# quantscious/finmlkit

Hardware: AMD Instinct MI355X
Metric: ticks/sec aggregated to bars (higher is better)
Workload: dtype f64

## Files before the change

finmlkit_amd/csrc/fmk_median.h:

```cpp
#pragma once
#include <math.h>

#include "fmk_common.h"
#include "fmk_dpp.h"

template <bool AF64> struct MedKey;
template <> struct MedKey<false> {
    typedef uint32_t K;
    static constexpr int BITS = 32;
    static constexpr K MAXK = 0xFFFFFFFFu;
    static constexpr K KEY_NEG_INF = 0x007FFFFFu;
    static constexpr K KEY_POS_INF = 0xFF800000u;
    __device__ static __forceinline__ K tokey(K u) { return (u & 0x80000000u) ? ~u : (u | 0x80000000u); }
    __device__ static __forceinline__ K load(const void *p, int64_t j) { return tokey(((const uint32_t *)p)[j]); }
    __device__ static __forceinline__ double value(K k)
    {
        uint32_t u = (k & 0x80000000u) ? (k & 0x7FFFFFFFu) : ~k;
        return (double)__uint_as_float(u);
    }
};
template <> struct MedKey<true> {
    typedef uint64_t K;
    static constexpr int BITS = 64;
    static constexpr K MAXK = 0xFFFFFFFFFFFFFFFFull;
    static constexpr K KEY_NEG_INF = 0x000FFFFFFFFFFFFFull;
    static constexpr K KEY_POS_INF = 0xFFF0000000000000ull;
    __device__ static __forceinline__ K tokey(K u) { return (u >> 63) ? ~u : (u | 0x8000000000000000ull); }
    __device__ static __forceinline__ K load(const void *p, int64_t j) { return tokey(((const uint64_t *)p)[j]); }
    __device__ static __forceinline__ double value(K k)
    {
        uint64_t u = (k >> 63) ? (k & 0x7FFFFFFFFFFFFFFFull) : ~k;
        return __longlong_as_double((long long)u);
    }
};

__device__ __forceinline__ int med_popc(bool p) { return __popcll(__ballot(p)); }

template <typename K>
__device__ __forceinline__ K med_wave_umin(K v)
{
#pragma unroll
    for (int o = 32; o > 0; o >>= 1) { K w = __shfl_xor(v, o, 64); v = w < v ? w : v; }
    return v;
}
template <typename K>
__device__ __forceinline__ K med_wave_umax(K v)
{
#pragma unroll
    for (int o = 32; o > 0; o >>= 1) { K w = __shfl_xor(v, o, 64); v = w > v ? w : v; }
    return v;
}

template <typename K>
__device__ __forceinline__ K med_bitonic64(K v, int lane)
{
#pragma unroll
    for (int k = 2; k <= 64; k <<= 1) {
#pragma unroll
        for (int j = k >> 1; j > 0; j >>= 1) {
            K w = __shfl_xor(v, j, 64);
            bool up = (lane & k) == 0;
            bool lower = (lane & j) == 0;
            K mn = w < v ? w : v, mx = w < v ? v : w;
            v = (lower == up) ? mn : mx;
        }
    }
    return v;
}

template <bool AF64, int NREG, bool EXACT = false>
struct MedBar {
    typedef MedKey<AF64> MK;
    typedef typename MK::K K;
    K key[NREG > 0 ? NREG : 1];
    const void *amount;
    int64_t start, cnt;
    int lane;

    __device__ __forceinline__ void load_all()
    {
        if constexpr (NREG > 0) {
            K raw[NREG];
#pragma unroll
            for (int r = 0; r < NREG; ++r) {
                const int64_t j = (int64_t)r * 64 + lane;
                raw[r] = 0;
                if (j < cnt) raw[r] = ((const K *)amount)[start + j];
            }
#pragma unroll
            for (int r = 0; r < NREG; ++r) asm volatile("" : "+v"(raw[r]));
#pragma unroll
            for (int r = 0; r < NREG; ++r) {
                const int64_t j = (int64_t)r * 64 + lane;
                key[r] = j < cnt ? MK::tokey(raw[r]) : MK::MAXK;
            }
        }
    }
    __device__ __forceinline__ bool maybe_invalid(int r) const { return !EXACT || r == NREG - 1; }
    __device__ __forceinline__ void minmax(K &mn, K &mx)
    {
        K a = MK::MAXK, b = 0;
        if constexpr (NREG > 0) {
#pragma unroll
            for (int r = 0; r < NREG; ++r) {
                const K k = key[r];
                a = k < a ? k : a;
                if (maybe_invalid(r)) b = (k != MK::MAXK && k > b) ? k : b;
                else b = k > b ? k : b;
            }
        } else {
            for (int64_t j = lane; j < cnt; j += 64) {
                K k = MK::load(amount, start + j);
                a = k < a ? k : a;
                b = k > b ? k : b;
            }
        }
        mn = med_wave_umin<K>(a);
        mx = med_wave_umax<K>(b);
    }
    __device__ __forceinline__ int64_t count_le(K pivot)
    {
        if constexpr (NREG > 0) {
            int c = 0;
#pragma unroll
            for (int r = 0; r < NREG; ++r) c += med_popc(key[r] <= pivot);
            return c;
        } else {
            int64_t c = 0;
            for (int64_t j = lane; j < cnt; j += 64) c += MK::load(amount, start + j) <= pivot;
            return fmk_wave_sum(c);
        }
    }
    __device__ __forceinline__ void split(K pivot, K &below, K &above)
    {
        K a = 0, b = MK::MAXK;
        if constexpr (NREG > 0) {
#pragma unroll
            for (int r = 0; r < NREG; ++r) {
                const K k = key[r];
                a = (k <= pivot && k > a) ? k : a;
                b = (k > pivot && k < b) ? k : b;
            }
        } else {
            for (int64_t j = lane; j < cnt; j += 64) {
                K k = MK::load(amount, start + j);
                a = (k <= pivot && k > a) ? k : a;
                b = (k > pivot && k < b) ? k : b;
            }
        }
        below = med_wave_umax<K>(a);
        above = med_wave_umin<K>(b);
    }
    __device__ __forceinline__ void inside_minmax(K lo, K hi, K &mn, K &mx)
    {
        K a = MK::MAXK, b = 0;
#pragma unroll
        for (int r = 0; r < (NREG > 0 ? NREG : 1); ++r) {
            const K k = key[r];
            const bool in = k > lo && k <= hi;
            a = (in && k < a) ? k : a;
            b = (in && k > b) ? k : b;
        }
        mn = med_wave_umin<K>(a);
        mx = med_wave_umax<K>(b);
    }
    __device__ __forceinline__ void compact(K lo, K hi, K *buf)
    {
        int base = 0;
        if constexpr (NREG > 0) {
#pragma unroll
            for (int r = 0; r < NREG; ++r) {
                K k = key[r];
                bool in = k > lo && k <= hi;
                uint64_t m = __ballot(in);
                int pos = base + __builtin_amdgcn_mbcnt_hi((uint32_t)(m >> 32), __builtin_amdgcn_mbcnt_lo((uint32_t)m, 0));
                if (in) buf[pos] = k;
                base += __popcll(m);
            }
        } else {
            for (int64_t j0 = 0; j0 < cnt; j0 += 64) {
                int64_t j = j0 + lane;
                K k = j < cnt ? MK::load(amount, start + j) : MK::MAXK;
                bool in = j < cnt && k > lo && k <= hi;
                uint64_t m = __ballot(in);
                int pos = base + __builtin_amdgcn_mbcnt_hi((uint32_t)(m >> 32), __builtin_amdgcn_mbcnt_lo((uint32_t)m, 0));
                if (in) buf[pos] = k;
                base += __popcll(m);
            }
        }
    }
};

template <bool AF64, int NREG, bool EXACT, bool SNAP = false>
__device__ __forceinline__ bool med_rank_pair(MedBar<AF64, NREG, EXACT> &bar, typename MedKey<AF64>::K *buf,
                                              int64_t k1, int64_t k2, typename MedKey<AF64>::K &v1,
                                              typename MedKey<AF64>::K &v2)
{
    typedef MedKey<AF64> MK;
    typedef typename MK::K K;
    const int lane = bar.lane;
    const int64_t cnt = bar.cnt;
    K mn, mx;
    bar.minmax(mn, mx);
    if (mn < MK::KEY_NEG_INF || mx > MK::KEY_POS_INF) return false;
    K lo = mn - 1, hi = mx;
    int64_t clo = 0, chi = cnt;
    for (int nstep = 0;; ++nstep) {
        if constexpr (SNAP && NREG > 0) {
            if (chi - clo > 64 && hi - lo > 1 && (nstep == 10 || nstep == 16 || nstep == 22)) {
                K mn_in, mx_in;
                bar.inside_minmax(lo, hi, mn_in, mx_in);
                hi = mx_in;
                lo = (mn_in == mx_in ? mx_in : mn_in) - 1;
                continue;
            }
        }
        if (chi - clo <= 64) {
            buf[lane] = MK::MAXK;
            __builtin_amdgcn_wave_barrier();
            bar.compact(lo, hi, buf);
            __builtin_amdgcn_wave_barrier();
            K v = med_bitonic64<K>(buf[lane], lane);
            __builtin_amdgcn_wave_barrier();
            v1 = __shfl(v, (int)(k1 - clo), 64);
            v2 = __shfl(v, (int)(k2 - clo), 64);
            break;
        }
        if (hi - lo == 1) { v1 = v2 = hi; break; }
        K pivot = lo + ((hi - lo) >> 1);
        int64_t c = bar.count_le(pivot);
        if (c > k2) { hi = pivot; chi = c; }
        else if (c <= k1) { lo = pivot; clo = c; }
        else {
            bar.split(pivot, v1, v2);
            break;
        }
    }
    return true;
}

template <bool AF64, int NREG, bool EXACT, bool SNAP = false>
__device__ __forceinline__ double med_search(MedBar<AF64, NREG, EXACT> &bar, typename MedKey<AF64>::K *buf)
{
    typedef MedKey<AF64> MK;
    typename MK::K v1, v2;
    const int64_t cnt = bar.cnt;
    if (!med_rank_pair<AF64, NREG, EXACT, SNAP>(bar, buf, (cnt - 1) >> 1, cnt >> 1, v1, v2)) return NAN;
    return (cnt & 1) ? MK::value(v1) : (MK::value(v1) + MK::value(v2)) / 2.0;
}

template <bool AF64, int NREG>
__device__ __forceinline__ double med_select(const void *amount, int64_t start, int64_t cnt, int lane,
                                             typename MedKey<AF64>::K *buf)
{
    MedBar<AF64, NREG, false> bar;
    bar.amount = amount; bar.start = start; bar.cnt = cnt; bar.lane = lane;
    bar.load_all();
    return med_search<AF64, NREG, false>(bar, buf);
}

#define MED_SEL_BITS 11
#define MED_SEL_BINS (1 << MED_SEL_BITS)
template <bool AF64, int THREADS>
__device__ __forceinline__ void med_block_select(const void *__restrict__ amount, int64_t start, int64_t cnt, int64_t rank0,
                                                 int64_t rank1, typename MedKey<AF64>::K &k1, typename MedKey<AF64>::K &k2,
                                                 bool &any_nan)
{
    typedef MedKey<AF64> MK;
    typedef typename MK::K K;
    constexpr int D = (MK::BITS + MED_SEL_BITS - 1) / MED_SEL_BITS;
    constexpr int PER = MED_SEL_BINS / THREADS;
    constexpr int NW = THREADS / 64;
    __shared__ unsigned hist[2][MED_SEL_BINS];
    __shared__ K s_prefix[2];
    __shared__ int64_t s_rank[2];
    __shared__ unsigned s_wsum[2][NW];
    __shared__ int s_nan;
    const int tid = threadIdx.x, lane = fmk_lane(), w = tid >> 6;
    __syncthreads();
    if (tid == 0) { s_prefix[0] = 0; s_prefix[1] = 0; s_rank[0] = rank0; s_rank[1] = rank1; s_nan = 0; }
    bool nan = false;
#pragma unroll 1
    for (int p = 0; p < D; ++p) {
#pragma unroll
        for (int q = 0; q < PER; ++q) { hist[0][tid + q * THREADS] = 0; hist[1][tid + q * THREADS] = 0; }
        __syncthreads();
        const K pre0 = s_prefix[0], pre1 = s_prefix[1];
        const int64_t rk0 = s_rank[0], rk1 = s_rank[1];
        const bool same = pre0 == pre1;
        const int rest = MK::BITS - MED_SEL_BITS * (p + 1);
        const int shift = rest > 0 ? rest : 0;
        const int width = rest >= 0 ? MED_SEL_BITS : MED_SEL_BITS + rest;
        const unsigned mask = (1u << width) - 1u;
        for (int64_t j = tid; j < cnt; j += THREADS) {
            const K k = MK::load(amount, start + j);
            if (p == 0) nan |= k < MK::KEY_NEG_INF || k > MK::KEY_POS_INF;
            const K hi = p == 0 ? (K)0 : (K)(k >> (shift + width));
            const unsigned d = (unsigned)(k >> shift) & mask;
            if (hi == pre0) atomicAdd(&hist[0][d], 1u);
            if (!same && hi == pre1) atomicAdd(&hist[1][d], 1u);
        }
        __syncthreads();
#pragma unroll
        for (int t = 0; t < 2; ++t) {
            const unsigned *hh = hist[same ? 0 : t];
            unsigned h[PER], tot = 0;
#pragma unroll
            for (int q = 0; q < PER; ++q) { h[q] = hh[tid * PER + q]; tot += h[q]; }
            unsigned inc = tot;
#pragma unroll
            for (int o = 1; o < 64; o <<= 1) { const unsigned v = __shfl_up(inc, o, 64); if (lane >= o) inc += v; }
            if (lane == 63) s_wsum[t][w] = inc;
            __syncthreads();
            unsigned base = 0;
            for (int k = 0; k < w; ++k) base += s_wsum[t][k];
            int64_t cum = (int64_t)base + inc - tot;
            const int64_t rk = t == 0 ? rk0 : rk1;
#pragma unroll
            for (int q = 0; q < PER; ++q) {
                if (cum <= rk && rk < cum + h[q]) {
                    s_prefix[t] = (K)(((t == 0 ? pre0 : pre1) << width) | (K)(tid * PER + q));
                    s_rank[t] = rk - cum;
                }
                cum += h[q];
            }
        }
        __syncthreads();
    }
    if (nan) s_nan = 1;
    __syncthreads();
    k1 = s_prefix[0]; k2 = s_prefix[1]; any_nan = s_nan != 0;
}

struct FuMed {
    uint32_t lo, hi;
    uint32_t width;
    int have;
};

__device__ __forceinline__ uint32_t fu_wave_umin(uint32_t v)
{
    return (uint32_t)fmk_dpp_reduce((int)(v ^ 0x80000000u), (int)0x7FFFFFFF, FmkOpMin()) ^ 0x80000000u;
}
__device__ __forceinline__ uint32_t fu_wave_umax(uint32_t v)
{
    return (uint32_t)fmk_dpp_reduce((int)(v ^ 0x80000000u), (int)0x80000000, FmkOpMax()) ^ 0x80000000u;
}

template <int R>
__device__ __forceinline__ double fu_median(const uint32_t (&key)[R], int cnt, int lane, bool maybe_nan, FuMed &med, uint32_t *buf)
{
    typedef MedKey<false> MK;
    const int k1 = (cnt - 1) >> 1, k2 = cnt >> 1;
    uint32_t lo = 0, hi = 0;
    int clo = 0, chi = cnt;
    bool inside = false;
    if (med.have && !maybe_nan) {
        int c1 = 0, c2 = 0;
#pragma unroll
        for (int i = 0; i < R; ++i) {
            c1 += med_popc(key[i] <= med.lo);
            c2 += med_popc(key[i] <= med.hi);
        }
        if (c1 <= k1 && k2 < c2) {
            inside = true; lo = med.lo; hi = med.hi; clo = c1; chi = c2;
            const int nc = c2 - c1;
            if (nc > 144) med.width -= med.width >> 2;
            else if (nc < 80) med.width += (med.width >> 2) + 1;
        }
    }
    if (!inside) {
        uint32_t a = MK::MAXK, bmax = 0;
#pragma unroll
        for (int i = 0; i < R; ++i) {
            const uint32_t k = key[i];
            a = k < a ? k : a;
            bmax = (k != MK::MAXK && k > bmax) ? k : bmax;
        }
        const uint32_t mn = fu_wave_umin(a), mx = fu_wave_umax(bmax);
        if (mn < MK::KEY_NEG_INF || mx > MK::KEY_POS_INF) { med.have = 0; return NAN; }
        lo = mn - 1; hi = mx; clo = 0; chi = cnt;
    }
    uint32_t v1 = 0, v2 = 0;
    bool found = false;
    while (chi - clo > 64) {
        if (hi - lo == 1) { v1 = v2 = hi; found = true; break; }
        const uint32_t pivot = lo + ((hi - lo) >> 1);
        int c = 0;
#pragma unroll
        for (int i = 0; i < R; ++i) c += med_popc(key[i] <= pivot);
        if (c > k2) { hi = pivot; chi = c; }
        else if (c <= k1) { lo = pivot; clo = c; }
        else {
            uint32_t a = 0, bb = MK::MAXK;
#pragma unroll
            for (int i = 0; i < R; ++i) {
                const uint32_t k = key[i];
                a = (k <= pivot && k > a) ? k : a;
                bb = (k > pivot && k < bb) ? k : bb;
            }
            v1 = fu_wave_umax(a); v2 = fu_wave_umin(bb);
            found = true;
            break;
        }
    }
    uint32_t cmin = 0, cmax = 0;
    if (!found) {
        buf[lane] = MK::MAXK;
        __builtin_amdgcn_wave_barrier();
        int base = 0;
#pragma unroll
        for (int i = 0; i < R; ++i) {
            const uint32_t k = key[i];
            const bool in = k > lo && k <= hi;
            const uint64_t m = __ballot(in);
            const int pos = base + (int)__builtin_amdgcn_mbcnt_hi((uint32_t)(m >> 32), __builtin_amdgcn_mbcnt_lo((uint32_t)m, 0));
            if (in) buf[pos] = k;
            base += __popcll(m);
        }
        __builtin_amdgcn_wave_barrier();
        const uint32_t c0 = buf[lane];
        __builtin_amdgcn_wave_barrier();
        if (!inside) {
            cmin = fu_wave_umin(c0);
            cmax = fu_wave_umax(lane < chi - clo ? c0 : 0u);
        }
        for (;;) {
            if (hi - lo == 1) { v1 = v2 = hi; break; }
            const uint32_t pivot = lo + ((hi - lo) >> 1);
            const int c = clo + med_popc(c0 <= pivot);
            if (c > k2) hi = pivot;
            else if (c <= k1) lo = pivot;
            else {
                v1 = fu_wave_umax(c0 <= pivot ? c0 : 0u);
                v2 = fu_wave_umin(c0 > pivot ? c0 : MK::MAXK);
                break;
            }
        }
    }
    if (!inside) {
        if (found) med.width = 64;
        else {
            const uint32_t wl = v1 - cmin, wh = cmax - v2;
            med.width = wl > wh ? wl : wh;
        }
        med.have = 1;
    }
    med.lo = v1 > med.width + 1 ? v1 - med.width - 1 : 0;
    med.hi = v2 < 0xFFFFFFFEu - med.width ? v2 + med.width : 0xFFFFFFFEu;
    return (cnt & 1) ? MK::value(v1) : (MK::value(v1) + MK::value(v2)) / 2.0;
}
```

finmlkit_amd/csrc/fmk_ohlcv.hip:

```cpp
#include <math.h>
#include <stdlib.h>

#include <utility>

#include "fmk_common.h"
#include "fmk_dpp.h"
#include "fmk_f32tie.h"
#include "fmk_median.h"

#define FMK_SMALL_NCH 21
#define FMK_PACKED_MAX_MEAN 64

struct OhlcvOut {
    double *open, *high, *low, *close;
    float *vol;
    double *vwap;
    int64_t *trades;
    double *median;
    unsigned long long *vol_redo;
};

__device__ __forceinline__ void ohlcv_empty(const OhlcvOut &o, int64_t b, const double *price, int64_t e, int64_t n)
{
    double p = price[fmk_wrap(e, n)];
// ... 89 lines not shown
        if constexpr (MED) {
            blo = brk[4 * q]; bhi = brk[4 * q + 1];
            mycand = cand + ((start - base) >> 2);
            cap = (int)((e - s) >> 2);
            if (tid == 0) { s_ncand = 0; s_nan = 0; }
            __syncthreads();
        }
        auto med_tick = [&](int64_t jj, bool in_bar) {
            if constexpr (MED) {
                const uint32_t raw = in_bar ? ((const uint32_t *)amount)[jj] : 0u;
                const uint32_t k = MedKey<false>::tokey(raw);
                nan |= in_bar && (k < MedKey<false>::KEY_NEG_INF || k > MedKey<false>::KEY_POS_INF);
                below += (in_bar && k < blo) ? 1 : 0;
                const bool inb = in_bar && k >= blo && k <= bhi;
                const uint64_t m = __ballot(inb);
                if (m) {
                    int base = 0;
                    if (lane == (int)__builtin_ctzll(m)) base = atomicAdd(&s_ncand, (int)__popcll(m));
                    base = __builtin_amdgcn_readlane(base, (int)__builtin_ctzll(m));
                    const int pos = base + (int)__builtin_amdgcn_mbcnt_hi((uint32_t)(m >> 32), __builtin_amdgcn_mbcnt_lo((uint32_t)m, 0));
                    if (inb && pos < cap) mycand[pos] = raw;
                }
            }
        };
        int64_t j = start + tid;
        for (; j + 3 * OH_WIDE_THREADS <= e; j += 4 * OH_WIDE_THREADS) {
            const double p0 = price[j], p1 = price[j + OH_WIDE_THREADS], p2 = price[j + 2 * OH_WIDE_THREADS],
                         p3 = price[j + 3 * OH_WIDE_THREADS];
            const double a0 = fmk_amt<AF64>(amount, j), a1 = fmk_amt<AF64>(amount, j + OH_WIDE_THREADS),
                         a2 = fmk_amt<AF64>(amount, j + 2 * OH_WIDE_THREADS), a3 = fmk_amt<AF64>(amount, j + 3 * OH_WIDE_THREADS);
            hi = fmax(fmax(hi, p0), fmax(p1, fmax(p2, p3)));
            lo = fmin(fmin(lo, p0), fmin(p1, fmin(p2, p3)));
            tv += a0; td += p0 * a0;
            tv += a1; td += p1 * a1;
            tv += a2; td += p2 * a2;
            tv += a3; td += p3 * a3;
            med_tick(j, true); med_tick(j + OH_WIDE_THREADS, true); med_tick(j + 2 * OH_WIDE_THREADS, true);
            med_tick(j + 3 * OH_WIDE_THREADS, true);
        }
        for (; j - tid <= e; j += OH_WIDE_THREADS) {
            const bool in_bar = j <= e;
            const int64_t jc = in_bar ? j : e;
            const double p0 = price[jc], a0 = in_bar ? fmk_amt<AF64>(amount, jc) : 0.0;
            hi = fmax(hi, p0);
            lo = fmin(lo, p0);
            tv += a0; td += in_bar ? p0 * a0 : 0.0;
            med_tick(jc, in_bar);
        }
        hi = fmk_dpp_reduce(hi, (double)-INFINITY, FmkOpMax());
        lo = fmk_dpp_reduce(lo, (double)INFINITY, FmkOpMin());
        tv = fmk_dpp_reduce(tv, 0.0, FmkOpAdd());
        td = fmk_dpp_reduce(td, 0.0, FmkOpAdd());
        if constexpr (MED) {
            below = fmk_dpp_reduce(below, (int64_t)0, FmkOpAdd());
            if (lane == 0) s_below[w] = below;
            if (__ballot(nan) != 0 && lane == 0) s_nan = 1;
        }
        if (lane == 0) { s_red[0][w] = hi; s_red[1][w] = lo; s_red[2][w] = tv; s_red[3][w] = td; }
        __syncthreads();
        if constexpr (MED) {
            if (tid == 0) {
                int64_t bl = 0;
                for (int k = 0; k < OH_WIDE_THREADS / 64; ++k) bl += s_below[k];
                res[3 * q] = bl; res[3 * q + 1] = s_ncand; res[3 * q + 2] = s_nan;
            }
        }
        if (w == 0) {
            hi = s_red[0][0]; lo = s_red[1][0]; tv = s_red[2][0]; td = s_red[3][0];
            for (int k = 1; k < OH_WIDE_THREADS / 64; ++k) {
                hi = fmax(hi, s_red[0][k]); lo = fmin(lo, s_red[1][k]); tv += s_red[2][k]; td += s_red[3][k];
            }
            ohlcv_finish<AF64>(o, b, price, start, e, hi, lo, tv, td, lane, true);
        }
        __syncthreads();
    }
}


struct OhlBracket { uint32_t blo, bhi; int ok; int pad; };
struct OhlCount { int64_t below; int64_t ncand; int64_t nan; };

__device__ __forceinline__ int ohl_stride(int64_t cnt) { return cnt <= 65536 ? 16 : (cnt <= ((int64_t)1 << 21) ? 64 : 256); }

__global__ __launch_bounds__(256) void k_bar_med_sample(const float *__restrict__ amount, const int64_t *__restrict__ ci,
                                                        const int64_t *__restrict__ list, const int *__restrict__ go,
                                                        float *__restrict__ samp, OhlBracket *__restrict__ brk, float g_scale,
                                                        int64_t base)
{
    if (go && *go == 0) return;
    const int64_t n_list = list[0];
    for (int64_t q = blockIdx.x; q < n_list; q += gridDim.x) {
        const int64_t b = list[1 + q], s0 = ci[b], e = ci[b + 1], start = s0 + 1, cnt = e - s0;
        const int stride = ohl_stride(cnt);
        const int64_t ns = cnt / stride;
        float *mine = samp + ((start - base) >> 4);
        for (int64_t j = threadIdx.x; j < ns; j += 256) mine[j] = amount[start + j * stride];
        __syncthreads();
        const int g = (int)(1.9f * g_scale * sqrtf((float)ns)) + 4;
        const int64_t r_lo = ns / 2 - g > 0 ? ns / 2 - g : 0, r_hi = ns / 2 + g < ns - 1 ? ns / 2 + g : ns - 1;
        uint32_t klo, khi;
        bool any_nan;
        med_block_select<false, 256>(mine, 0, ns, r_lo, r_hi, klo, khi, any_nan);
        if (threadIdx.x == 0) brk[q] = OhlBracket{klo, khi, any_nan ? 0 : 1, 0};
        __syncthreads();
    }
}

__global__ __launch_bounds__(256) void k_bar_med_finish(const int64_t *__restrict__ ci, const int64_t *__restrict__ list,
                                                        const int *__restrict__ go, const uint32_t *__restrict__ cand,
                                                        const OhlCount *__restrict__ res, int64_t *__restrict__ fallback,
                                                        double *__restrict__ o_median, int64_t base)
{
    if (go && *go == 0) return;
    typedef MedKey<false> MK;
    const int64_t n_list = list[0];
    for (int64_t q = blockIdx.x; q < n_list; q += gridDim.x) {
        const int64_t b = list[1 + q], s0 = ci[b], e = ci[b + 1], start = s0 + 1, cnt = e - s0;
        const OhlCount r = res[q];
        const int64_t k1 = (cnt - 1) >> 1, k2 = cnt >> 1, cap = cnt >> 2;
        if (r.nan) { if (threadIdx.x == 0) o_median[b] = NAN; continue; }
        if (!(r.below <= k1 && k2 < r.below + r.ncand && r.ncand <= cap)) {
            if (threadIdx.x == 0) fallback[1 + atomicAdd((unsigned long long *)fallback, 1ULL)] = b;
            continue;
        }
        uint32_t v1, v2;
        bool any_nan;
        med_block_select<false, 256>(cand + ((start - base) >> 2), 0, r.ncand, k1 - r.below, k2 - r.below, v1, v2, any_nan);
        if (threadIdx.x == 0) o_median[b] = (cnt & 1) ? MK::value(v1) : (MK::value(v1) + MK::value(v2)) / 2.0;
        __syncthreads();
    }
}

int fmk_median_long_list_launch(fmk_ctx *ctx, const void *d_amount, const int64_t *d_close_idx, const int64_t *d_list, double *d_median);

__global__ __launch_bounds__(256) void k_list_span(const int64_t *__restrict__ ci, const int64_t *__restrict__ list, int64_t *__restrict__ out)
{
    __shared__ long long s_lo, s_hi;
    if (threadIdx.x == 0) { s_lo = INT64_MAX; s_hi = 0; }
    __syncthreads();
    const int64_t n_list = list[0];
    long long lo = INT64_MAX, hi = 0;
    for (int64_t q = threadIdx.x; q < n_list; q += 256) {
        const int64_t b = list[1 + q];
        const long long s = ci[b] + 1, e = ci[b + 1] + 1;
        lo = s < lo ? s : lo;
        hi = e > hi ? e : hi;
    }
    atomicMin(&s_lo, lo);
    atomicMax(&s_hi, hi);
    __syncthreads();
    if (threadIdx.x == 0) { out[0] = n_list; out[1] = n_list ? s_lo : 0; out[2] = n_list ? s_hi : 0; }
}

template <bool AF64>
static int oh_wide_launch(fmk_ctx *ctx, const double *p, const void *a, const int64_t *ci, int64_t nb, int64_t n, const int *go,
                          const OhlcvOut &o, int *median_done = nullptr, int64_t wide_min = OH_WIDE_MIN)
{
    int64_t *list = nullptr;
    FMK_TRY(fmk_long_bar_list(ctx, ci, nb, n, wide_min, go, &list));
    if constexpr (!AF64) {
        if (o.median && median_done) {
            const int64_t cap = n / wide_min + 2;
            int64_t base = 0, span = n;
            if (!ctx->enqueue_only) {
                int64_t *d_span = ctx->d_mail->ohlcv.span, h_span[3];
                k_list_span<<<1, 256, 0, ctx->stream>>>(ci, list, d_span);
                FMK_LAUNCH_CHECK(ctx);
                FMK_TRY(fmk_read_back(ctx, h_span, d_span, sizeof h_span));
                if (h_span[0] == 0) {
                    FMK_TRY(fmk_free(ctx, list));
                    *median_done = 1;
                    return FMK_OK;
                }
                base = h_span[1] & ~(int64_t)15;
                span = h_span[2] - base;
            }
            float *samp = nullptr;
            uint32_t *cand = nullptr;
            OhlBracket *brk = nullptr;
            int64_t *res = nullptr, *fallback = nullptr;
            int rc = fmk_alloc(ctx, (size_t)((span >> 4) + 64) * 4, (void **)&samp);
            if (rc == FMK_OK) rc = fmk_alloc(ctx, (size_t)((span >> 2) + 64) * 4, (void **)&cand);
            if (rc == FMK_OK) rc = fmk_alloc(ctx, (size_t)cap * sizeof(OhlBracket), (void **)&brk);
            if (rc == FMK_OK) rc = fmk_alloc(ctx, (size_t)cap * 3 * 8, (void **)&res);
            if (rc == FMK_OK) rc = fmk_alloc(ctx, (size_t)(cap + 1) * 8, (void **)&fallback);
            const bool have_scratch = rc == FMK_OK;
            hipError_t le = hipSuccess;
            if (have_scratch) le = hipMemsetAsync(fallback, 0, 8, ctx->stream);
            if (have_scratch && le == hipSuccess) {
                const char *gv = getenv("FMK_WIDE_MED_GSCALE");
                k_bar_med_sample<<<(unsigned)(ctx->n_cu * 4), 256, 0, ctx->stream>>>((const float *)a, ci, list, go, samp, brk,
                                                                                   gv ? (float)atof(gv) : 1.0f, base);
                k_bar_ohlcv_wide<false, true><<<(unsigned)(ctx->n_cu * 2), OH_WIDE_THREADS, 0, ctx->stream>>>(
                    p, a, ci, list, go, o, (const uint32_t *)brk, cand, res, base);
                k_bar_med_finish<<<(unsigned)(ctx->n_cu * 4), 256, 0, ctx->stream>>>(ci, list, go, cand, (const OhlCount *)res, fallback,
                                                                                   o.median, base);
                le = hipGetLastError();
                rc = FMK_OK;
                if (le == hipSuccess) rc = fmk_median_long_list_launch(ctx, a, ci, fallback, o.median);
            }
            if (samp) (void)fmk_free(ctx, samp);
            if (cand) (void)fmk_free(ctx, cand);
            if (brk) (void)fmk_free(ctx, brk);
            if (res) (void)fmk_free(ctx, res);
            if (fallback) (void)fmk_free(ctx, fallback);
            if (have_scratch) {
                (void)fmk_free(ctx, list);
                FMK_TRY(rc);
                FMK_HIP(ctx, le);
                *median_done = 1;
                return FMK_OK;
            }
            if (rc != FMK_E_NOMEM) { (void)fmk_free(ctx, list); FMK_TRY(rc); }
        }
    }
    k_bar_ohlcv_wide<AF64><<<(unsigned)(ctx->n_cu * 2), OH_WIDE_THREADS, 0, ctx->stream>>>(p, a, ci, list, go, o);
    const hipError_t le = hipGetLastError();
    FMK_TRY(fmk_free(ctx, list));
    FMK_HIP(ctx, le);
    return FMK_OK;
}

template <bool AF64>
__global__ __launch_bounds__(256) void k_bar_ohlcv(const double *__restrict__ price,
                                                   const void *__restrict__ amount,
                                                   const int64_t *__restrict__ ci, int64_t nb, int64_t n,
                                                   int64_t min_cnt, const int *__restrict__ go, OhlcvOut o,
                                                   int64_t skip_lo = 0, int64_t skip_hi = 0)
{
    if (go && *go == 0) return;
    const int lane = fmk_lane();
    const int wpb = blockDim.x >> 6;
    const int64_t wave0 = (int64_t)blockIdx.x * wpb + fmk_uniform((int)(threadIdx.x >> 6));
    const int64_t nwaves = (int64_t)gridDim.x * wpb;
    auto do_bar = [&](int64_t b, int64_t s, int64_t e) {
        if (e <= s) {
            if (lane == 0) ohlcv_empty(o, b, price, e, n);
            return;
        }
        if (e - s > OH_WIDE_MIN) return;
        if (e - s > skip_lo && e - s <= skip_hi) return;
        const int64_t start = s + 1;
        double hi = -INFINITY, lo = INFINITY, tv = 0.0, td = 0.0;
        int64_t j = start + lane;
        for (; j + 192 <= e; j += 256) {
            double p0 = price[j], p1 = price[j + 64], p2 = price[j + 128], p3 = price[j + 192];
            double a0 = fmk_amt<AF64>(amount, j), a1 = fmk_amt<AF64>(amount, j + 64);
            double a2 = fmk_amt<AF64>(amount, j + 128), a3 = fmk_amt<AF64>(amount, j + 192);
            hi = fmax(fmax(hi, p0), fmax(p1, fmax(p2, p3)));
            lo = fmin(fmin(lo, p0), fmin(p1, fmin(p2, p3)));
            tv += a0; td += p0 * a0;
            tv += a1; td += p1 * a1;
            tv += a2; td += p2 * a2;
            tv += a3; td += p3 * a3;
        }
        for (; j <= e; j += 64) {
            double p0 = price[j];
            double a0 = fmk_amt<AF64>(amount, j);
            hi = fmax(hi, p0);
            lo = fmin(lo, p0);
            tv += a0; td += p0 * a0;
        }
        ohlcv_finish<AF64>(o, b, price, start, e, hi, lo, tv, td, lane);
    };
    if (min_cnt > 0) {
        const int64_t ngroups = (nb + 63) >> 6;
        for (int64_t g = wave0; g < ngroups; g += nwaves) {
            const int64_t bl = g * 64 + lane;
            int64_t s_l = 0, e_l = 0;
            if (bl < nb) { s_l = ci[bl]; e_l = ci[bl + 1]; }
            unsigned long long todo = __builtin_amdgcn_ballot_w64(bl < nb && e_l - s_l > min_cnt);
            while (todo) {
                const int bit = fmk_uniform((int)__builtin_ctzll(todo));
                todo &= todo - 1;
                do_bar(g * 64 + bit, fmk_readlane(s_l, bit), fmk_readlane(e_l, bit));
            }
        }
        return;
    }
    for (int64_t b = wave0; b < nb; b += nwaves) do_bar(b, fmk_uniform(ci[b]), fmk_uniform(ci[b + 1]));
}

template <bool AF64, int NCH, bool EXACT, bool MEDIAN>
__device__ __forceinline__ void small_bar(const double *__restrict__ price, const void *__restrict__ amount,
                                          int64_t b, int64_t start, int64_t e, int64_t cnt, int lane,
                                          typename MedKey<AF64>::K *buf, const OhlcvOut &o)
{
    typedef MedKey<AF64> MK;
    typedef typename MK::K K;
    const double *pb = price + start;
    const K *ab = (const K *)amount + start;
    const unsigned last = (unsigned)(cnt - 1);
    double p[NCH];
    K araw[NCH];
#pragma unroll
    for (int c = 0; c < NCH; ++c) {
        unsigned idx = (unsigned)(c * 64 + lane);
        if (!EXACT || c == NCH - 1) idx = idx < last ? idx : last;
        p[c] = pb[idx];
        araw[c] = ab[idx];
    }
    double hi = -INFINITY, lo = INFINITY, tv = 0.0, td = 0.0;
    MedBar<AF64, NCH, EXACT> bar;
#pragma unroll
    for (int c = 0; c < NCH; ++c) {
        double a;
        if constexpr (AF64) a = __longlong_as_double((long long)araw[c]);
        else a = (double)__uint_as_float(araw[c]);
        hi = fmax(hi, p[c]);
        lo = fmin(lo, p[c]);
        const double pa = p[c] * a;
        if (!EXACT || c == NCH - 1) {
            const bool valid = (unsigned)(c * 64 + lane) <= last;
            tv += valid ? a : 0.0;
            td += valid ? pa : 0.0;
            if constexpr (MEDIAN) bar.key[c] = valid ? MK::tokey(araw[c]) : MK::MAXK;
        } else {
            tv += a;
            td += pa;
            if constexpr (MEDIAN) bar.key[c] = MK::tokey(araw[c]);
        }
    }
    ohlcv_finish<AF64>(o, b, price, start, e, hi, lo, tv, td, lane);
    if constexpr (MEDIAN) {
        bar.amount = amount; bar.start = start; bar.cnt = cnt; bar.lane = lane;
        const double m = med_search<AF64, NCH, EXACT>(bar, buf);
        if (lane == 0) o.median[b] = m;
    }
}

template <bool AF64, bool MEDIAN, int MAXNCH = FMK_SMALL_NCH>
__global__ __launch_bounds__(256, (MAXNCH <= 4 ? 8 : MAXNCH <= 10 ? 6 : 4)) void k_bar_ohlcv_small(const double *__restrict__ price,
                                                            const void *__restrict__ amount,
                                                            const int64_t *__restrict__ ci, int64_t nb, int64_t n,
                                                            int *__restrict__ saw_long, OhlcvOut o)
{
    typedef typename MedKey<AF64>::K K;
    __shared__ K sbuf[4][64];
    const int lane = fmk_lane();
    const int wib = fmk_uniform((int)(threadIdx.x >> 6));
    const int wpb = blockDim.x >> 6;
    const int64_t wave0 = (int64_t)blockIdx.x * wpb + wib;
    const int64_t nwaves = (int64_t)gridDim.x * wpb;
    K *buf = sbuf[wib];
    for (int64_t b = wave0; b < nb; b += nwaves) {
        const int64_t s = fmk_uniform(ci[b]);
        const int64_t e = fmk_uniform(ci[b + 1]);
        const int64_t cnt = e - s;
        if (cnt > 64 * MAXNCH) {
            if (lane == 0 && __hip_atomic_load(saw_long, __ATOMIC_RELAXED, __HIP_MEMORY_SCOPE_AGENT) == 0)
                __hip_atomic_store(saw_long, 1, __ATOMIC_RELAXED, __HIP_MEMORY_SCOPE_AGENT);
            continue;
        }
        if (cnt <= 0) {
            if (lane == 0) ohlcv_empty(o, b, price, e, n);
            continue;
        }
        const int64_t start = s + 1;
        const int nch = (int)((cnt + 63) >> 6);
        if constexpr (MAXNCH <= 4) {
            switch (nch) {
            case 1: small_bar<AF64, 1, true, MEDIAN>(price, amount, b, start, e, cnt, lane, buf, o); break;
            case 2: small_bar<AF64, 2, true, MEDIAN>(price, amount, b, start, e, cnt, lane, buf, o); break;
            case 3: small_bar<AF64, 3, true, MEDIAN>(price, amount, b, start, e, cnt, lane, buf, o); break;
            default: small_bar<AF64, 4, true, MEDIAN>(price, amount, b, start, e, cnt, lane, buf, o); break;
            }
        } else if constexpr (MAXNCH <= 10) {
            switch (nch) {
            case 1: small_bar<AF64, 1, true, MEDIAN>(price, amount, b, start, e, cnt, lane, buf, o); break;
            case 2: small_bar<AF64, 2, true, MEDIAN>(price, amount, b, start, e, cnt, lane, buf, o); break;
            case 3: small_bar<AF64, 3, true, MEDIAN>(price, amount, b, start, e, cnt, lane, buf, o); break;
            case 4: small_bar<AF64, 4, true, MEDIAN>(price, amount, b, start, e, cnt, lane, buf, o); break;
            case 5: small_bar<AF64, 5, true, MEDIAN>(price, amount, b, start, e, cnt, lane, buf, o); break;
            case 6: small_bar<AF64, 6, true, MEDIAN>(price, amount, b, start, e, cnt, lane, buf, o); break;
            case 7: small_bar<AF64, 7, true, MEDIAN>(price, amount, b, start, e, cnt, lane, buf, o); break;
            case 8: small_bar<AF64, 8, true, MEDIAN>(price, amount, b, start, e, cnt, lane, buf, o); break;
            case 9: small_bar<AF64, 9, true, MEDIAN>(price, amount, b, start, e, cnt, lane, buf, o); break;
            default: small_bar<AF64, 10, true, MEDIAN>(price, amount, b, start, e, cnt, lane, buf, o); break;
            }
        } else {
            switch (nch) {
            case 11: small_bar<AF64, 11, true, MEDIAN>(price, amount, b, start, e, cnt, lane, buf, o); break;
            case 12: small_bar<AF64, 12, true, MEDIAN>(price, amount, b, start, e, cnt, lane, buf, o); break;
            case 13: small_bar<AF64, 13, true, MEDIAN>(price, amount, b, start, e, cnt, lane, buf, o); break;
            case 14: small_bar<AF64, 14, true, MEDIAN>(price, amount, b, start, e, cnt, lane, buf, o); break;
            case 15: small_bar<AF64, 15, true, MEDIAN>(price, amount, b, start, e, cnt, lane, buf, o); break;
            case 16: small_bar<AF64, 16, true, MEDIAN>(price, amount, b, start, e, cnt, lane, buf, o); break;
            case 17: small_bar<AF64, 17, true, MEDIAN>(price, amount, b, start, e, cnt, lane, buf, o); break;
            case 18: small_bar<AF64, 18, true, MEDIAN>(price, amount, b, start, e, cnt, lane, buf, o); break;
            case 19: small_bar<AF64, 19, true, MEDIAN>(price, amount, b, start, e, cnt, lane, buf, o); break;
            case 20: small_bar<AF64, 20, true, MEDIAN>(price, amount, b, start, e, cnt, lane, buf, o); break;
            case 21: small_bar<AF64, 21, true, MEDIAN>(price, amount, b, start, e, cnt, lane, buf, o); break;
            default:
                if (nch <= 1) small_bar<AF64, 1, true, MEDIAN>(price, amount, b, start, e, cnt, lane, buf, o);
                else if (nch <= 4) small_bar<AF64, 4, false, MEDIAN>(price, amount, b, start, e, cnt, lane, buf, o);
                else if (nch <= 10) small_bar<AF64, 10, false, MEDIAN>(price, amount, b, start, e, cnt, lane, buf, o);
                else small_bar<AF64, 16, false, MEDIAN>(price, amount, b, start, e, cnt, lane, buf, o);
            }
        }
    }
}

struct TbFuse {
    const int64_t *ts;
    int64_t e0, d;
    int64_t t_first, t_last;
    int64_t *clock, *idx;
};


template <int NCH>
__device__ __forceinline__ void median_bar(const void *__restrict__ amount, int64_t b, int64_t start, int64_t cnt, int lane,
                                           uint32_t *buf, double *__restrict__ o_median, FuMed &med)
{
    typedef MedKey<false> MK;
    const uint32_t *ab = (const uint32_t *)amount + start;
    const unsigned last = (unsigned)(cnt - 1);
    uint32_t key[NCH];
    bool nan = false;
#pragma unroll
    for (int c = 0; c < NCH; ++c) {
        unsigned idx = (unsigned)(c * 64 + lane);
        if (c == NCH - 1) idx = idx < last ? idx : last;
        const uint32_t raw = ab[idx];
        nan |= (raw & 0x7FFFFFFFu) > 0x7F800000u;
        key[c] = (c < NCH - 1 || (unsigned)(c * 64 + lane) <= last) ? MK::tokey(raw) : MK::MAXK;
    }
    const bool any_nan = __ballot(nan) != 0;
    double m;
    if (any_nan) { m = NAN; med.have = 0; }
    else m = fu_median<NCH>(key, (int)cnt, lane, false, med, buf);
    if (lane == 0) o_median[b] = m;
}

__global__ __launch_bounds__(256) void k_bar_median_small(const float *__restrict__ amount, const int64_t *__restrict__ ci,
                                                          int64_t nb, int *__restrict__ saw_long, double *__restrict__ o_median)
{
    __shared__ uint32_t sbuf[4][64];
    const int lane = fmk_lane();
    const int wib = fmk_uniform((int)(threadIdx.x >> 6));
    const int64_t wave0 = (int64_t)blockIdx.x * 4 + wib;
    const int64_t nwaves = (int64_t)gridDim.x * 4;
    uint32_t *buf = sbuf[wib];
    FuMed med;
    med.lo = med.hi = 0; med.width = 64; med.have = 0;
    for (int64_t b = wave0; b < nb; b += nwaves) {
        const int64_t s = fmk_uniform(ci[b]);
        const int64_t e = fmk_uniform(ci[b + 1]);
        const int64_t cnt = e - s;
        if (cnt > 64 * FMK_SMALL_NCH) {
            if (lane == 0 && __hip_atomic_load(saw_long, __ATOMIC_RELAXED, __HIP_MEMORY_SCOPE_AGENT) == 0)
                __hip_atomic_store(saw_long, 1, __ATOMIC_RELAXED, __HIP_MEMORY_SCOPE_AGENT);
            continue;
        }
        if (cnt <= 0) { if (lane == 0) o_median[b] = 0.0; continue; }
        const int64_t start = s + 1;
        switch ((int)((cnt + 63) >> 6)) {
#define FMK_MB(N) case N: median_bar<N>(amount, b, start, cnt, lane, buf, o_median, med); break;
            FMK_MB(1) FMK_MB(2) FMK_MB(3) FMK_MB(4) FMK_MB(5) FMK_MB(6) FMK_MB(7) FMK_MB(8) FMK_MB(9) FMK_MB(10) FMK_MB(11)
            FMK_MB(12) FMK_MB(13) FMK_MB(14) FMK_MB(15) FMK_MB(16) FMK_MB(17) FMK_MB(18) FMK_MB(19) FMK_MB(20)
#undef FMK_MB
        default: median_bar<21>(amount, b, start, cnt, lane, buf, o_median, med); break;
        }
    }
}

int fmk_median_small_launch(fmk_ctx *ctx, const float *d_amount, const int64_t *d_close_idx, int64_t nb, double *d_median,
                            int64_t n_ticks)
{
    int *saw_long = &ctx->d_mail->ohlcv.saw_long;
    FMK_HIP(ctx, hipMemsetAsync(saw_long, 0, sizeof(int), ctx->stream));
    int64_t blocks = fmk_ceil_div(nb, 4);
    const int64_t cap = (int64_t)ctx->n_cu * 64;
    if (blocks > cap) blocks = cap;
    if (blocks < 1) blocks = 1;
    k_bar_median_small<<<(unsigned)blocks, 256, 0, ctx->stream>>>(d_amount, d_close_idx, nb, saw_long, d_median);
    FMK_LAUNCH_CHECK(ctx);
    return fmk_median_launch(ctx, d_amount, 0, d_close_idx, nb, 64 * FMK_SMALL_NCH, saw_long, d_median, n_ticks);
}


template <int I, int J, int K, int N>
__device__ __forceinline__ void lb_ce(uint32_t (&r)[N])
{
    constexpr int l = I ^ J;
    if constexpr (l > I) {
        const uint32_t a = r[I], b = r[l];
        const uint32_t mn = a < b ? a : b, mx = a < b ? b : a;
        if constexpr ((I & K) == 0) { r[I] = mn; r[l] = mx; }
        else { r[I] = mx; r[l] = mn; }
    }
}
template <int J, int K, int N, int... I>
__device__ __forceinline__ void lb_stage(uint32_t (&r)[N], std::integer_sequence<int, I...>)
{
    (lb_ce<I, J, K, N>(r), ...);
}
template <int J, int K, int N>
__device__ __forceinline__ void lb_js(uint32_t (&r)[N])
{
    lb_stage<J, K, N>(r, std::make_integer_sequence<int, N>{});
    if constexpr (J > 1) lb_js<J / 2, K, N>(r);
}
template <int K, int N>
__device__ __forceinline__ void lb_ks(uint32_t (&r)[N])
{
    lb_js<K / 2, K, N>(r);
    if constexpr (K < N) lb_ks<K * 2, N>(r);
}
template <int N>
__device__ __forceinline__ void lb_sort(uint32_t (&r)[N]) { lb_ks<2, N>(r); }

template <int N, int... I>
__device__ __forceinline__ uint32_t lb_pick_seq(const uint32_t (&r)[N], int idx, std::integer_sequence<int, I...>)
{
    uint32_t v = r[0];
    ((v = idx == I ? r[I] : v), ...);
    return v;
}
template <int N>
__device__ __forceinline__ uint32_t lb_pick(const uint32_t (&r)[N], int idx)
{
    return lb_pick_seq<N>(r, idx, std::make_integer_sequence<int, N>{});
}

template <bool MEDIAN, int N, int K, int NR>
__device__ __forceinline__ void lb_block(const double *tp, const uint32_t *ta, int off, int L, int Lmax, int zero_at, double &hi, double &lo,
                                         double (&lv)[3], double (&ld)[3], double &tv, double &td, uint32_t (&r)[NR])
{
    typedef MedKey<false> MK;
    constexpr int j0 = 8 * K;
    double cv = 0.0, cd = 0.0;
    if (j0 < Lmax) {
        double p[8];
        uint32_t raw[8];
#pragma unroll
        for (int q = 0; q < 8; ++q) {
            const int at = j0 + q < L ? off + j0 + q : zero_at;
            p[q] = tp[at];
            raw[q] = ta[at];
        }
        double xv[8], xd[8];
#pragma unroll
        for (int q = 0; q < 8; ++q) {
            const bool in = j0 + q < L;
            const double a = (double)__uint_as_float(raw[q]);
            if (in) {
                hi = p[q] > hi ? p[q] : hi;
                lo = p[q] < lo ? p[q] : lo;
            }
            xv[q] = a;
            xd[q] = p[q] * a;
            if constexpr (MEDIAN) r[j0 + q] = in ? MK::tokey(raw[q]) : MK::MAXK;
        }
        cv = ((xv[0] + xv[1]) + (xv[2] + xv[3])) + ((xv[4] + xv[5]) + (xv[6] + xv[7]));
        cd = ((xd[0] + xd[1]) + (xd[2] + xd[3])) + ((xd[4] + xd[5]) + (xd[6] + xd[7]));
    } else if constexpr (MEDIAN) {
#pragma unroll
        for (int q = 0; q < 8; ++q) r[j0 + q] = MK::MAXK;
    }
    constexpr int NB = N / 8;
    if constexpr ((K & 1) == 0 && NB > 1) { lv[0] = cv; ld[0] = cd; }
    else {
        if constexpr (NB > 1) { cv = lv[0] + cv; cd = ld[0] + cd; }
        if constexpr ((K & 2) == 0 && NB > 2) { lv[1] = cv; ld[1] = cd; }
        else {
            if constexpr (NB > 2) { cv = lv[1] + cv; cd = ld[1] + cd; }
            if constexpr ((K & 4) == 0 && NB > 4) { lv[2] = cv; ld[2] = cd; }
            else {
                if constexpr (NB > 4) { cv = lv[2] + cv; cd = ld[2] + cd; }
                tv = cv; td = cd;
            }
        }
    }
    __builtin_amdgcn_sched_barrier(0);
    asm volatile("" ::: "memory");
    if constexpr (K + 1 < NB) lb_block<MEDIAN, N, K + 1, NR>(tp, ta, off, L, Lmax, zero_at, hi, lo, lv, ld, tv, td, r);
}

template <bool MEDIAN, int N>
__device__ __forceinline__ void lb_bar(const double *tp, const uint32_t *ta, int off, int L, int zero_at, double &hi, double &lo,
                                       double &tv, double &td, double &med)
{
    typedef MedKey<false> MK;
    uint32_t r[MEDIAN ? N : 1];
    double lv[3] = {0.0, 0.0, 0.0}, ld[3] = {0.0, 0.0, 0.0};
    const int Lmax = fmk_dpp_reduce(L, 0, FmkOpMax());
    lb_block<MEDIAN, N, 0, (MEDIAN ? N : 1)>(tp, ta, off, L, Lmax, zero_at, hi, lo, lv, ld, tv, td, r);
    if constexpr (MEDIAN) {
        lb_sort<N>(r);
        const uint32_t v1 = lb_pick<N>(r, (L - 1) >> 1), v2 = lb_pick<N>(r, L >> 1);
        const uint32_t kmx = lb_pick<N>(r, L > 0 ? L - 1 : 0), kmn = r[0];
        if (kmn < MK::KEY_NEG_INF || kmx > MK::KEY_POS_INF) med = NAN;
        else med = (L & 1) ? MK::value(v1) : (MK::value(v1) + MK::value(v2)) / 2.0;
    }
}

template <bool MEDIAN, int LB_TILE>
__global__ __launch_bounds__(128) void k_bar_ohlcv_lanes(const double *__restrict__ price, const float *__restrict__ amount,
                                                         const int64_t *__restrict__ ci, int64_t nb, int64_t n,
                                                         int *__restrict__ saw_long, OhlcvOut o)
{
    __shared__ double s_p[2][LB_TILE + 2];
    __shared__ uint32_t s_a[2][LB_TILE + 2];
    __shared__ int64_t s_ci[2][66];
    const int lane = fmk_lane();
    const int w = fmk_uniform((int)(threadIdx.x >> 6));
    double *tp = s_p[w];
    uint32_t *ta = s_a[w];
    if (lane == 0) { tp[LB_TILE] = 0.0; ta[LB_TILE] = 0u; }
    const int64_t ngroups = (nb + 63) >> 6;
    const int64_t nwaves = (int64_t)gridDim.x * 2;
    for (int64_t g = (int64_t)blockIdx.x * 2 + w; g < ngroups; g += nwaves) {
        const int64_t B0 = g * 64;
        const int nbg = (int)(nb - B0 < 64 ? nb - B0 : 64);
        __builtin_amdgcn_wave_barrier();
        if (lane <= nbg) s_ci[w][lane] = ci[B0 + lane];
        if (lane == 0 && nbg == 64) s_ci[w][64] = ci[B0 + 64];
        __builtin_amdgcn_wave_barrier();
        int bl = 0;
        while (bl < nbg) {
            const int64_t s0 = s_ci[w][bl];
            const int idx = bl + 1 + lane;
            const bool valid = idx <= nbg;
            const int64_t e_l = valid ? s_ci[w][idx] : INT64_MAX;
            const int64_t s_l = valid ? s_ci[w][idx - 1] : 0;
            const int m = __popcll(__ballot(valid && e_l - s0 <= LB_TILE));
            if (m == 0) {
                if (lane == 0 && __hip_atomic_load(saw_long, __ATOMIC_RELAXED, __HIP_MEMORY_SCOPE_AGENT) == 0)
// ... 838 lines not shown
```

Measured before the change: 448.8 billion.

## Replace bitonic tail sort with rank search and DPP wave min/max

Wave-wide unsigned min/max reductions now go through the DPP reduction helper instead of xor-shuffle loops. The final stage of the median search no longer bitonic-sorts the last 64 candidates; it runs a popcount bisection over the compacted keys (shared med_tail). In the small-bar OHLCV kernel, per-lane key min/max is computed in the same loop that builds the keys, avoiding a second pass over registers. The aim is to cut shuffle-heavy work in median computation, at the cost of a data-dependent bisection loop in the tail.

```diff
diff --git a/finmlkit_amd/csrc/fmk_median.h b/finmlkit_amd/csrc/fmk_median.h
--- a/finmlkit_amd/csrc/fmk_median.h
+++ b/finmlkit_amd/csrc/fmk_median.h
@@ -39,16 +39,45 @@
 template <typename K>
 __device__ __forceinline__ K med_wave_umin(K v)
 {
-#pragma unroll
-    for (int o = 32; o > 0; o >>= 1) { K w = __shfl_xor(v, o, 64); v = w < v ? w : v; }
-    return v;
+    if constexpr (sizeof(K) == 4)
+        return (K)((uint32_t)fmk_dpp_reduce((int)((uint32_t)v ^ 0x80000000u), (int)0x7FFFFFFF, FmkOpMin()) ^ 0x80000000u);
+    else
+        return (K)((uint64_t)fmk_dpp_reduce((int64_t)((uint64_t)v ^ 0x8000000000000000ull), (int64_t)0x7FFFFFFFFFFFFFFFll, FmkOpMin()) ^
+                   0x8000000000000000ull);
 }
 template <typename K>
 __device__ __forceinline__ K med_wave_umax(K v)
 {
-#pragma unroll
-    for (int o = 32; o > 0; o >>= 1) { K w = __shfl_xor(v, o, 64); v = w > v ? w : v; }
-    return v;
+    if constexpr (sizeof(K) == 4)
+        return (K)((uint32_t)fmk_dpp_reduce((int)((uint32_t)v ^ 0x80000000u), (int)0x80000000, FmkOpMax()) ^ 0x80000000u);
+    else
+        return (K)((uint64_t)fmk_dpp_reduce((int64_t)((uint64_t)v ^ 0x8000000000000000ull), (int64_t)0x8000000000000000ull, FmkOpMax()) ^
+                   0x8000000000000000ull);
+}
+
+template <typename K>
+__device__ __forceinline__ void med_tail(K c0, K lo, K hi, int r1, int r2, int nin, K &v1, K &v2)
+{
+    constexpr K MAXK = (K)~(K)0;
+    int bot = 0, top = nin;
+    for (;;) {
+        if (hi - lo == 1) { v1 = v2 = hi; break; }
+        if (top - bot == r2 - r1 + 1) {
+            const bool in = c0 > lo && c0 <= hi;
+            v1 = med_wave_umin<K>(in ? c0 : MAXK);
+            v2 = med_wave_umax<K>(in ? c0 : (K)0);
+            break;
+        }
+        const K pivot = lo + ((hi - lo) >> 1);
+        const int c = med_popc(c0 <= pivot);
+        if (c > r2) { hi = pivot; top = c; }
+        else if (c <= r1) { lo = pivot; bot = c; }
+        else {
+            v1 = med_wave_umax<K>(c0 <= pivot ? c0 : (K)0);
+            v2 = med_wave_umin<K>(c0 > pivot ? c0 : MAXK);
+            break;
+        }
+    }
 }
 
 template <typename K>
@@ -97,9 +126,9 @@
         }
     }
     __device__ __forceinline__ bool maybe_invalid(int r) const { return !EXACT || r == NREG - 1; }
-    __device__ __forceinline__ void minmax(K &mn, K &mx)
-    {
-        K a = MK::MAXK, b = 0;
+    __device__ __forceinline__ void lane_minmax(K &a, K &b)
+    {
+        a = MK::MAXK; b = 0;
         if constexpr (NREG > 0) {
 #pragma unroll
             for (int r = 0; r < NREG; ++r) {
@@ -115,8 +144,6 @@
                 b = k > b ? k : b;
             }
         }
-        mn = med_wave_umin<K>(a);
-        mx = med_wave_umax<K>(b);
     }
     __device__ __forceinline__ int64_t count_le(K pivot)
     {
@@ -193,15 +220,15 @@
 
 template <bool AF64, int NREG, bool EXACT, bool SNAP = false>
 __device__ __forceinline__ bool med_rank_pair(MedBar<AF64, NREG, EXACT> &bar, typename MedKey<AF64>::K *buf,
-                                              int64_t k1, int64_t k2, typename MedKey<AF64>::K &v1,
+                                              int64_t k1, int64_t k2, typename MedKey<AF64>::K lane_mn,
+                                              typename MedKey<AF64>::K lane_mx, typename MedKey<AF64>::K &v1,
                                               typename MedKey<AF64>::K &v2)
 {
     typedef MedKey<AF64> MK;
     typedef typename MK::K K;
     const int lane = bar.lane;
     const int64_t cnt = bar.cnt;
-    K mn, mx;
-    bar.minmax(mn, mx);
+    const K mn = med_wave_umin<K>(lane_mn), mx = med_wave_umax<K>(lane_mx);
     if (mn < MK::KEY_NEG_INF || mx > MK::KEY_POS_INF) return false;
     K lo = mn - 1, hi = mx;
     int64_t clo = 0, chi = cnt;
@@ -220,10 +247,9 @@
             __builtin_amdgcn_wave_barrier();
             bar.compact(lo, hi, buf);
             __builtin_amdgcn_wave_barrier();
-            K v = med_bitonic64<K>(buf[lane], lane);
+            const K c0 = buf[lane];
             __builtin_amdgcn_wave_barrier();
-            v1 = __shfl(v, (int)(k1 - clo), 64);
-            v2 = __shfl(v, (int)(k2 - clo), 64);
+            med_tail<K>(c0, lo, hi, (int)(k1 - clo), (int)(k2 - clo), (int)(chi - clo), v1, v2);
             break;
         }
         if (hi - lo == 1) { v1 = v2 = hi; break; }
@@ -238,6 +264,15 @@
     }
     return true;
 }
+template <bool AF64, int NREG, bool EXACT, bool SNAP = false>
+__device__ __forceinline__ bool med_rank_pair(MedBar<AF64, NREG, EXACT> &bar, typename MedKey<AF64>::K *buf,
+                                              int64_t k1, int64_t k2, typename MedKey<AF64>::K &v1,
+                                              typename MedKey<AF64>::K &v2)
+{
+    typename MedKey<AF64>::K a, b;
+    bar.lane_minmax(a, b);
+    return med_rank_pair<AF64, NREG, EXACT, SNAP>(bar, buf, k1, k2, a, b, v1, v2);
+}
 
 template <bool AF64, int NREG, bool EXACT, bool SNAP = false>
 __device__ __forceinline__ double med_search(MedBar<AF64, NREG, EXACT> &bar, typename MedKey<AF64>::K *buf)
@@ -246,6 +281,16 @@
     typename MK::K v1, v2;
     const int64_t cnt = bar.cnt;
     if (!med_rank_pair<AF64, NREG, EXACT, SNAP>(bar, buf, (cnt - 1) >> 1, cnt >> 1, v1, v2)) return NAN;
+    return (cnt & 1) ? MK::value(v1) : (MK::value(v1) + MK::value(v2)) / 2.0;
+}
+template <bool AF64, int NREG, bool EXACT>
+__device__ __forceinline__ double med_search(MedBar<AF64, NREG, EXACT> &bar, typename MedKey<AF64>::K *buf,
+                                             typename MedKey<AF64>::K lane_mn, typename MedKey<AF64>::K lane_mx)
+{
+    typedef MedKey<AF64> MK;
+    typename MK::K v1, v2;
+    const int64_t cnt = bar.cnt;
+    if (!med_rank_pair<AF64, NREG, EXACT, false>(bar, buf, (cnt - 1) >> 1, cnt >> 1, lane_mn, lane_mx, v1, v2)) return NAN;
     return (cnt & 1) ? MK::value(v1) : (MK::value(v1) + MK::value(v2)) / 2.0;
 }
 
@@ -338,14 +383,8 @@
     int have;
 };
 
-__device__ __forceinline__ uint32_t fu_wave_umin(uint32_t v)
-{
-    return (uint32_t)fmk_dpp_reduce((int)(v ^ 0x80000000u), (int)0x7FFFFFFF, FmkOpMin()) ^ 0x80000000u;
-}
-__device__ __forceinline__ uint32_t fu_wave_umax(uint32_t v)
-{
-    return (uint32_t)fmk_dpp_reduce((int)(v ^ 0x80000000u), (int)0x80000000, FmkOpMax()) ^ 0x80000000u;
-}
+__device__ __forceinline__ uint32_t fu_wave_umin(uint32_t v) { return med_wave_umin<uint32_t>(v); }
+__device__ __forceinline__ uint32_t fu_wave_umax(uint32_t v) { return med_wave_umax<uint32_t>(v); }
 
 template <int R>
 __device__ __forceinline__ double fu_median(const uint32_t (&key)[R], int cnt, int lane, bool maybe_nan, FuMed &med, uint32_t *buf)
@@ -425,18 +464,7 @@
             cmin = fu_wave_umin(c0);
             cmax = fu_wave_umax(lane < chi - clo ? c0 : 0u);
         }
-        for (;;) {
-            if (hi - lo == 1) { v1 = v2 = hi; break; }
-            const uint32_t pivot = lo + ((hi - lo) >> 1);
-            const int c = clo + med_popc(c0 <= pivot);
-            if (c > k2) hi = pivot;
-            else if (c <= k1) lo = pivot;
-            else {
-                v1 = fu_wave_umax(c0 <= pivot ? c0 : 0u);
-                v2 = fu_wave_umin(c0 > pivot ? c0 : MK::MAXK);
-                break;
-            }
-        }
+        med_tail<uint32_t>(c0, lo, hi, k1 - clo, k2 - clo, chi - clo, v1, v2);
     }
     if (!inside) {
         if (found) med.width = 64;
diff --git a/finmlkit_amd/csrc/fmk_ohlcv.hip b/finmlkit_amd/csrc/fmk_ohlcv.hip
--- a/finmlkit_amd/csrc/fmk_ohlcv.hip
+++ b/finmlkit_amd/csrc/fmk_ohlcv.hip
@@ -415,6 +415,7 @@
     }
     double hi = -INFINITY, lo = INFINITY, tv = 0.0, td = 0.0;
     MedBar<AF64, NCH, EXACT> bar;
+    K kmn = MK::MAXK, kmx = 0;
 #pragma unroll
     for (int c = 0; c < NCH; ++c) {
         double a;
@@ -427,17 +428,27 @@
             const bool valid = (unsigned)(c * 64 + lane) <= last;
             tv += valid ? a : 0.0;
             td += valid ? pa : 0.0;
-            if constexpr (MEDIAN) bar.key[c] = valid ? MK::tokey(araw[c]) : MK::MAXK;
+            if constexpr (MEDIAN) {
+                const K k = valid ? MK::tokey(araw[c]) : MK::MAXK;
+                bar.key[c] = k;
+                kmn = k < kmn ? k : kmn;
+                kmx = (k != MK::MAXK && k > kmx) ? k : kmx;
+            }
         } else {
             tv += a;
             td += pa;
-            if constexpr (MEDIAN) bar.key[c] = MK::tokey(araw[c]);
+            if constexpr (MEDIAN) {
+                const K k = MK::tokey(araw[c]);
+                bar.key[c] = k;
+                kmn = k < kmn ? k : kmn;
+                kmx = k > kmx ? k : kmx;
+            }
         }
     }
     ohlcv_finish<AF64>(o, b, price, start, e, hi, lo, tv, td, lane);
     if constexpr (MEDIAN) {
         bar.amount = amount; bar.start = start; bar.cnt = cnt; bar.lane = lane;
-        const double m = med_search<AF64, NCH, EXACT>(bar, buf);
+        const double m = med_search<AF64, NCH, EXACT>(bar, buf, kmn, kmx);
         if (lane == 0) o.median[b] = m;
     }
 }
```

New measurement: 460.8 billion, median of 4. 2.7% higher.
